# AzheeeQAQ/Game-of-life-distributed

Measured on AMD Instinct MI355X. Metric: cell-updates/sec (GCUPS) at 1/2/4/8 MI355X; % of HBM roofline, higher is better.
Workload: dtype u32 bit-sliced (1 bit/cell)

## Files before the change

### game-of-life-distributed_amd/csrc/gol_kernels.hip

```cpp
#include "gol_kernels.h"
#include "gol_bits.h"
#include "gol_layout.h"

#include <algorithm>
#include <climits>
#include <type_traits>
#include <utility>

namespace golk {
#ifndef GOL_LOOP_PAD
#define GOL_LOOP_PAD 0
#endif
#ifndef GOL_FILL_PHASES
#define GOL_FILL_PHASES 4
#endif

template <typename F, int... I>
__device__ __forceinline__ void static_for_impl(F &&f, std::integer_sequence<int, I...>) {
    (f(std::integral_constant<int, I>()), ...);
}
template <int N, typename F>
__device__ __forceinline__ void static_for(F &&f) {
    static_for_impl(f, std::make_integer_sequence<int, N>());
}
// ... 696 lines not shown
    unit_pr<D, (KQ + 0 + LO) & 1, WPL>(LO, x0, sh, st, x1, nx);
    sh = nx;
    static_for<D - LO>([&](auto t_tag) {
        constexpr int t = LO + decltype(t_tag)::value;
        parity_fix<2>();
        if constexpr (t + 1 < D) {
            unit_pr<D, (KQ + 1 + t) & 1, WPL>(t, x1, sh, st, x0, nx);
            sh = nx;
            unit_pr<D, (KQ + 0 + t + 1) & 1, WPL>(t + 1, x0, sh, st, x2, nx);
            sh = nx;
            unit_pr<D, (KQ + 2 + t) & 1, WPL>(t, x2, sh, st, x1, nx);
            sh = nx;
        } else {
            unit_pr<D, (KQ + 1 + t) & 1, WPL>(t, x1, sh, st, x2, nx);
            sh = nx;
            xn = vmov_even(n0);
            __builtin_amdgcn_sched_barrier(0);
            unit_pr<D, (KQ + 2 + t) & 1, WPL>(t, x2, sh, st, xn, nx);
            sh = nx;
        }
    });
}
template <int D, int KQ, int WPL>
__device__ __forceinline__ void push_group_pr(Lanes<WPL> &x0, Lanes<WPL> &x1, Lanes<WPL> &x2, PairSt<D, WPL> &st,
                                              Shifted &sh, const Lanes<WPL> &n0, Lanes<WPL> &xn) {
    push_group_pr_hi<D, KQ, 0, WPL>(x0, x1, x2, st, sh, n0, xn);
}

template <int D, int KQ, int WPL>
__device__ __forceinline__ void pr_enter(const uint32_t (&h0)[3][D][WPL], const uint32_t (&h1)[3][D][WPL],
                                         const uint32_t (&cc)[3][D][WPL], PairSt<D, WPL> &st) {
#pragma unroll
    for (int t = 0; t < D; ++t)
#pragma unroll
        for (int k = 0; k < WPL; ++k) {
            st.c[t][k] = cc[2][t][k];
            if (((KQ + t) & 1) == 1) {
                st.a0[t][k] = h0[1][t][k];
                st.a1[t][k] = h1[1][t][k];
                st.b0[t][k] = h0[2][t][k];
                st.b1[t][k] = h1[2][t][k];
            } else {
                pair_sum(h0[1][t][k], h1[1][t][k], h0[2][t][k], h1[2][t][k], st.p0[t][k], st.p1[t][k], st.p2[t][k]);
                st.a0[t][k] = h0[2][t][k];
                st.a1[t][k] = h1[2][t][k];
            }
        }
}
template <int D, int KQ, int WPL>
__device__ __forceinline__ void pr_leave(const PairSt<D, WPL> &st, uint32_t (&h0)[3][D][WPL],
                                         uint32_t (&h1)[3][D][WPL], uint32_t (&cc)[3][D][WPL]) {
#pragma unroll
    for (int t = 0; t < D; ++t)
#pragma unroll
        for (int k = 0; k < WPL; ++k) {
            cc[2][t][k] = st.c[t][k];
            if (((KQ + t) & 1) == 1) {
                h0[1][t][k] = st.a0[t][k];
                h1[1][t][k] = st.a1[t][k];
                h0[2][t][k] = st.b0[t][k];
                h1[2][t][k] = st.b1[t][k];
            } else {
                h0[2][t][k] = st.a0[t][k];
                h1[2][t][k] = st.a1[t][k];
                pair_unsum(st.p0[t][k], st.p1[t][k], st.a0[t][k], st.a1[t][k], h0[1][t][k], h1[1][t][k]);
            }
        }
}

template <int D, int LO, int WPL>
__device__ __forceinline__ void push_group_hi(Lanes<WPL> &x0, Lanes<WPL> &x1, Lanes<WPL> &x2,
                                              uint32_t (&h0)[3][D][WPL], uint32_t (&h1)[3][D][WPL],
                                              uint32_t (&cc)[3][D][WPL]) {
    parity_fix<1>();
#pragma unroll
    for (int s = LO; s < D + 2; ++s) {
        parity_fix<2>();
        if (s < D) stage<D, 0, WPL>(s, x0, h0, h1, cc);
        if (s - 1 >= LO && s - 1 < D) stage<D, 1, WPL>(s - 1, x1, h0, h1, cc);
        if (s - 2 >= LO) stage<D, 2, WPL>(s - 2, x2, h0, h1, cc);
    }
}

template <int D, int WPL, bool HALF = false, bool PR = false>
__device__ __forceinline__ uint32_t stream_skew(const StepArgs &a, int ab, int eb, int tile, bool self,
                                                uint32_t *exp_mine, const uint32_t *exp_next, int *flag_mine,
                                                int *flag_next, unsigned *error, unsigned long long *phase_tr,
                                                int dr = 0) {
    using SP = SkewPlan<D>;
    constexpr int ROW = 64 * WPL;
    constexpr int TV = HALF ? kHalfTileValid : kTileValid;
    const int lane = threadIdx.x & 63;
    const int hl = HALF ? (lane & 31) : lane;
    const int rofs = (HALF && lane >= 32) ? dr : 0;
    const int Ww = a.Ww;
    const int S = eb - ab;
    const int t0 = tile * TV * WPL;
    int col = (t0 + WPL * (hl - 1)) % Ww;
    if (col < 0) col += Ww;
    const bool keep = hl >= 1 && hl <= TV && (t0 + WPL * (hl - 1)) < Ww;
    int r = ab + rofs + a.in.off;
    const int wrap = a.in.wrap > 0 ? a.in.wrap : INT_MAX;
    if (a.in.wrap > 0) {
        r %= a.in.wrap;
        if (r < 0) r += a.in.wrap;
    }
    const uint32_t *__restrict__ src = a.src + col;
    auto load_next = [&]() -> Lanes<WPL> {
        const Lanes<WPL> v = load_row<WPL>(src + (size_t)(a.in.base + min(r, a.in.rmax)) * Ww);
        r = (r + 1 == wrap) ? 0 : r + 1;
        return v;
    };
    const __amdgpu_buffer_rsrc_t brs = __builtin_amdgcn_make_buffer_rsrc(
        a.dst + (size_t)(a.dst_base + ab + D) * Ww, (short)0, (S + (HALF ? dr : 0)) * Ww * 4, 0x00020000);
    const int clo = a.count_lo - (ab + D + rofs), chi = a.count_hi - (ab + D + rofs);
    const int colw = col + rofs * Ww;
    uint32_t cnt = 0;
    auto emit = [&](const Lanes<WPL> &y, int oi) {
        const bool ok = keep && (unsigned)oi < (unsigned)S;
        const int off = ok ? (oi * Ww + colw) * 4 : INT_MAX;
        if constexpr (WPL == 1)
            __builtin_amdgcn_raw_buffer_store_b32(y.w[0], brs, off, 0, GOL_SKEW_STORE_CPOL);
        else if constexpr (WPL == 2)
            __builtin_amdgcn_raw_buffer_store_b64((__attribute__((ext_vector_type(2))) unsigned){y.w[0], y.w[1]}, brs,
                                                  off, 0, GOL_SKEW_STORE_CPOL);
        else
            __builtin_amdgcn_raw_buffer_store_b128(
                (__attribute__((ext_vector_type(4))) unsigned){y.w[0], y.w[1], y.w[2], y.w[3]}, brs, off, 0,
                GOL_SKEW_STORE_CPOL);
        uint32_t pc = 0;
#pragma unroll
        for (int k = 0; k < WPL; ++k) pc += __builtin_popcount(y.w[k]);
        cnt += (ok && oi >= clo && oi < chi) ? pc : 0u;
    };
    auto hook = [&](int s, int k, const Lanes<WPL> &x) {
        if (s % SP::STEP != 0 || s == 0 || s / SP::STEP > SP::NPH) return;
        const int j = s / SP::STEP - 1;
        const int m = k - 2 * SP::P(j);
        const int row = (unsigned)m < (unsigned)SP::NROWS(j) ? SP::BASE(j) + m : SP::NEXP;
        put_lanes<WPL>(exp_mine + row * ROW, x.w);
    };

    uint32_t h0[3][D][WPL], h1[3][D][WPL], cc[3][D][WPL];
#pragma unroll
    for (int s = 0; s < 3; ++s)
#pragma unroll
        for (int t = 0; t < D; ++t)
#pragma unroll
            for (int k = 0; k < WPL; ++k) h0[s][t][k] = h1[s][t][k] = cc[s][t][k] = 0u;

    Lanes<WPL> x0 = vmov(load_next()), x1 = vmov(load_next()), x2 = vmov(load_next());
    int k = 0;
    [[maybe_unused]] unsigned long long wt0 = 0, wmain = 0, nmain = 0, wfill = 0, nfill = 0;
    auto fill = [&](auto a_tag) {
        constexpr int A = decltype(a_tag)::value;
        for (; A == D ? k <= 2 * D - 1 : (k + 2) / 2 <= A - 1; k += 3) {
            const Lanes<WPL> n0 = load_next(), n1 = load_next(), n2 = load_next();
            __builtin_amdgcn_sched_barrier(0);
            Lanes<WPL> y0 = x0, y1 = x1, y2 = x2;
            push_group_exp<D, A, WPL>(y0, y1, y2, h0, h1, cc, k, hook);
            if constexpr (A == D) {
                emit(y0, k - 2 * D);
                emit(y1, k + 1 - 2 * D);
                emit(y2, k + 2 - 2 * D);
            }
            __builtin_amdgcn_sched_barrier(0);
            if constexpr (GOL_SKEW_WAIT_TRACE) wt0 = __builtin_amdgcn_s_memrealtime();
            x0 = vmov(n0);
            x1 = vmov(n1);
            x2 = vmov(n2);
            if constexpr (GOL_SKEW_WAIT_TRACE) {
                asm volatile("s_waitcnt vmcnt(0)" ::: "memory");
                wfill += __builtin_amdgcn_s_memrealtime() - wt0;
                ++nfill;
            }
        }
    };
    static_for<SP::NPH>([&](auto j) { fill(std::integral_constant<int, SP::P(decltype(j)::value)>()); });
    fill(std::integral_constant<int, D>());
    if (phase_tr && lane == 0) phase_tr[0] = (unsigned long long)__builtin_amdgcn_s_memrealtime();
    asm volatile("s_waitcnt lgkmcnt(0)" ::: "memory");
    if (lane == 0) __hip_atomic_store(flag_mine, 1, __ATOMIC_RELAXED, __HIP_MEMORY_SCOPE_WORKGROUP);

    Lanes<WPL> q0, q1, q2;
#pragma unroll
    for (int i = 0; i < WPL; ++i) q0.w[i] = q1.w[i] = q2.w[i] = 0u;
    int qoi = -8;
    [[maybe_unused]] PairSt<D, WPL> st;
    [[maybe_unused]] Shifted sh = {0u, 0u};
    const int kmain = S + (self ? 2 * D : 2 * SP::P(0));
    for (int i = 0; i < GOL_LOOP_PAD; ++i) asm volatile("s_nop 0");
    if constexpr (PR) {
        constexpr int KSTART = 3 * ((2 * D + 2) / 3);
        static_assert(KSTART % 6 == 0, "the pair main loop starts at an even push");
        {
            pr_enter<D, 0, WPL>(h0, h1, cc, st);
            sh = row_shifts<WPL>(x0);
            for (; k < kmain; k += 6) {
                {
                    const Lanes<WPL> n0 = load_next(), n1 = load_next(), n2 = load_next();
                    emit(q0, qoi);
                    emit(q1, qoi + 1);
                    emit(q2, qoi + 2);
                    __builtin_amdgcn_sched_barrier(0);
                    Lanes<WPL> y0 = x0, y1 = x1, y2 = x2;
                    Lanes<WPL> xn;
                    push_group_pr<D, 0, WPL>(y0, y1, y2, st, sh, n0, xn);
                    q0 = y0;
                    q1 = y1;
                    q2 = y2;
                    qoi = k - 2 * D;
                    __builtin_amdgcn_sched_barrier(0);
                    x0 = xn;
                    if constexpr (HALF) x1 = vmov(n1); else x1 = vmov_even(n1);
                    x2 = vmov(n2);
                }
// ... 69 lines not shown
            static_for<SP::NPH>([&](auto j) {
                constexpr int J = decltype(j)::value;
                if (J > 0 && d >= 2 * SP::P(J)) base = SP::BASE(J) - 2 * SP::P(J);
            });
            const int top = SP::NEXP - 1;
            y0 = get_lanes<WPL>(exp_next + min(base + d, top) * ROW);
            y1 = get_lanes<WPL>(exp_next + min(base + d + 1, top) * ROW);
            y2 = get_lanes<WPL>(exp_next + min(base + d + 2, top) * ROW);
        };
        {
            Lanes<WPL> n0, n1, n2;
            imports(k, n0, n1, n2);
            x0 = vmov(n0);
            x1 = vmov(n1);
            x2 = vmov(n2);
            if constexpr (PR && D % 3 == 0) sh = row_shifts<WPL>(x0);
        }
        auto drain_pr = [&](auto kq_tag, auto lo_tag) {
            constexpr int KQ = decltype(kq_tag)::value, LO = decltype(lo_tag)::value;
            Lanes<WPL> n0, n1, n2;
            imports(k + 3, n0, n1, n2);
            __builtin_amdgcn_sched_barrier(0);
            Lanes<WPL> y0 = x0, y1 = x1, y2 = x2;
            Lanes<WPL> xn;
            push_group_pr_hi<D, KQ, LO, WPL>(y0, y1, y2, st, sh, n0, xn);
            parity_fix<1>();
            emit(q0, qoi);
            emit(q1, qoi + 1);
            emit(q2, qoi + 2);
            q0 = y0;
            q1 = y1;
            q2 = y2;
            qoi = k - 2 * D;
            __builtin_amdgcn_sched_barrier(0);
            x0 = xn;
            x1 = vmov(n1);
            x2 = vmov(n2);
            k += 3;
        };
        auto drain = [&](auto lo_tag, int kend) {
            constexpr int LO = decltype(lo_tag)::value;
            if constexpr (PR && D % 3 == 0) {
                if constexpr (LO == SP::P(SP::NPH - 1) && D - LO <= 6) {
                    static_for<(D - LO) / 3>([&](auto) {
                        drain_pr(std::integral_constant<int, 0>(), lo_tag);
                        drain_pr(std::integral_constant<int, 1>(), lo_tag);
                    });
                    return;
                }
                while (k < kend) {
                    drain_pr(std::integral_constant<int, 0>(), lo_tag);
                    drain_pr(std::integral_constant<int, 1>(), lo_tag);
                }
                return;
            }
            for (; k < kend; k += 3) {
                Lanes<WPL> n0, n1, n2;
                imports(k + 3, n0, n1, n2);
                __builtin_amdgcn_sched_barrier(0);
                Lanes<WPL> y0 = x0, y1 = x1, y2 = x2;
                push_group_hi<D, LO, WPL>(y0, y1, y2, h0, h1, cc);
                __builtin_amdgcn_sched_barrier(0);
                emit(q0, qoi);
                emit(q1, qoi + 1);
                emit(q2, qoi + 2);
                q0 = y0;
                q1 = y1;
                q2 = y2;
                qoi = k - 2 * D;
                __builtin_amdgcn_sched_barrier(0);
                x0 = vmov(n0);
                x1 = vmov(n1);
                x2 = vmov(n2);
            }
        };
        static_for<SP::NPH>([&](auto j) {
            constexpr int J = decltype(j)::value;
            drain(std::integral_constant<int, SP::P(J)>(), S + 2 * (J + 1 < SP::NPH ? SP::P(J + 1) : D));
        });
    }
    emit(q0, qoi);
    emit(q1, qoi + 1);
    emit(q2, qoi + 2);
    return cnt;
}

template <int D, int WPL, bool HALF = false, bool PR = false>
__global__ __launch_bounds__(512) void gol_skew_kernel(SkewArgs p) {
    using SP = SkewPlan<D>;
    constexpr int ROW = 64 * WPL;
    __shared__ uint32_t s_exp[8][(SP::NEXP + 1) * ROW];
    __shared__ int s_flag[8];
    __shared__ unsigned long long s_cnt;
    const int lane = threadIdx.x & 63;
    const int w = __builtin_amdgcn_readfirstlane(threadIdx.x >> 6);
    const int sy = 8 / p.tx;
    const int tcols = (p.tiles_x + p.tx - 1) / p.tx;
    const int stack = blockIdx.x / tcols, tc = blockIdx.x - stack * tcols;
    const int tile = tc * p.tx + w % p.tx, pos = w / p.tx;
    if (lane == 0) s_flag[w] = 0;
    if (threadIdx.x == 0) s_cnt = 0;
    __syncthreads();
    if (tile >= p.tiles_x) return;
    if (p.prio_young && w >= 4) __builtin_amdgcn_s_setprio(1);
    const int L = HALF ? p.base.rows_out / 2 : p.base.rows_out;
    const int A0 = (int)((int64_t)stack * L / p.nst) - D, E0 = (int)((int64_t)(stack + 1) * L / p.nst) - D;
    const int64_t Ls = (int64_t)(E0 - A0) + p.hcap;
    int cum = 0, tot = 0;
    for (int q = 0; q < sy; ++q) {
        tot += p.wgt[q];
        cum += q < pos ? p.wgt[q] : 0;
    }
    const bool bottom = pos == sy - 1;
    constexpr int G = PR ? 6 : 3;
    const int ab = A0 + (int)(Ls * cum / tot) / G * G;
    const int eb = bottom ? E0 : A0 + (int)(Ls * (cum + p.wgt[pos]) / tot) / G * G;
    const long long t_start = p.trace ? (long long)__builtin_amdgcn_s_memrealtime() : 0;
    const uint32_t cnt = stream_skew<D, WPL, HALF, PR>(p.base, ab, eb, tile, bottom, s_exp[w], bottom ? nullptr : s_exp[w + p.tx],
                                             &s_flag[w], bottom ? nullptr : &s_flag[w + p.tx], p.error,
                                             (p.trace && blockIdx.x < 1024) ? p.trace + 8 + 2 * (blockIdx.x * 64 + 16 + w)
                                                                            : nullptr,
                                             L);
    if (p.trace && lane == 0 && blockIdx.x < 1024) {
        p.trace[8 + 2 * (blockIdx.x * 64 + w)] = (unsigned long long)t_start;
        p.trace[8 + 2 * (blockIdx.x * 64 + w) + 1] = (unsigned long long)__builtin_amdgcn_s_memrealtime();
    }
    if (p.base.alive) wg_count(p.base.alive, &s_cnt, cnt, sy * min(p.tx, p.tiles_x - tc * p.tx));
}

__host__ __device__ constexpr int persist_waves(int depth, int wpl) { return depth * wpl <= 16 ? 16 : 8; }

#ifndef GOL_PERSIST_WG_COUNT
#define GOL_PERSIST_WG_COUNT 1
#endif
template <int D, int WPL, int NW>
__global__ __launch_bounds__(NW * 64) void gol_persist_kernel(PersistArgs p) {
    const int lane = threadIdx.x & 63;
    const int w = __builtin_amdgcn_readfirstlane(threadIdx.x >> 6);
    const int b = blockIdx.x;
    const int wx = b % p.cols, wy = b / p.cols;
    const int tile = wx * p.wg_tx + w % p.wg_tx;
    int r0, band, dir = 1;
    const int ry = w / p.wg_tx;
    const bool paired = p.paired != 0;
    if (paired) {
        const int hr = p.wg_sy / 2;
        r0 = wy * p.wg_sy * p.S + 2 * (ry % hr) * p.S;
        band = 2 * p.S;
        dir = ry < hr ? 1 : -1;
    } else if (p.S_old > 0) {
        const int hr = p.wg_sy / 2;
        const int base = wy * p.wg_sy * p.S;
        r0 = base + (ry < hr ? ry * p.S_old : hr * p.S_old + (ry - hr) * p.S_young);
        band = ry < hr ? p.S_old : p.S_young;
        if (ry == p.wg_sy - 1) band = base + p.wg_sy * p.S - r0;
    } else {
        r0 = (wy * p.wg_sy + ry) * p.S;
        band = p.S;
    }
    const int rows_here = (tile < p.tiles_x && r0 < p.base.rows_out) ? min(band, p.base.rows_out - r0) : 0;

    int nb = b;
    if (lane < 9) {
        const int ny = (wy + lane / 3 - 1 + p.wg_y) % p.wg_y;
        const int nx = (wx + lane % 3 - 1 + p.cols) % p.cols;
        nb = ny * p.cols + nx;
    }
    __shared__ int s_abort;
    __shared__ int s_claim[2][NW / 2];
#if GOL_PERSIST_WG_COUNT
    __shared__ unsigned long long s_cnt;
    if (threadIdx.x == 0) s_cnt = 0;
#endif
    if (threadIdx.x == 0) s_abort = 0;
    if (paired && w < NW / 2 && lane == 0) s_claim[0][w] = rows_here;
    __syncthreads();

    uint32_t cnt = 0;
    long long tr_wait = 0, tr_band = 0, tr_max = 0;
    const long long tr_t0 = (long long)__builtin_amdgcn_s_memrealtime();
    for (int j = 0; j < p.J; ++j) {
        const long long tr_w0 = (long long)__builtin_amdgcn_s_memrealtime();
        if (j > 0) {
            if (w == NW - 1) {
                const long long t_start = (long long)__builtin_amdgcn_s_memrealtime();
                for (;;) {
                    const unsigned v = __hip_atomic_load(&p.progress[nb], __ATOMIC_RELAXED, __HIP_MEMORY_SCOPE_AGENT);
                    if (__all(v >= (unsigned)j)) break;
                    const unsigned err = __hip_atomic_load(p.error, __ATOMIC_RELAXED, __HIP_MEMORY_SCOPE_AGENT);
                    if (err || (long long)__builtin_amdgcn_s_memrealtime() - t_start > p.timeout_ticks) {
                        if (lane == 0) {
                            atomicOr(p.error, 1u);
                            s_abort = 1;
                        }
                        break;
                    }
                    __builtin_amdgcn_s_sleep(2);
                }
                if (lane == 0) __builtin_amdgcn_fence(__ATOMIC_ACQUIRE, "agent");
                asm volatile("s_waitcnt vmcnt(0)" ::: "memory");
            }
            __syncthreads();
            if (s_abort) return;
        }
        const long long tr_b0 = (long long)__builtin_amdgcn_s_memrealtime();
        tr_wait += tr_b0 - tr_w0;
        StepArgs a = p.base;
        const bool odd = ((p.first + j) & 1) != 0;
        a.src = odd ? p.buf1 : p.buf0;
        a.dst = odd ? p.buf0 : p.buf1;
// ... 451 lines not shown
    }
    return n;
}

hipError_t launch_lds_band(const LdsBandArgs &p, int wpl, hipStream_t s) {
    const size_t bytes = (size_t)lds_band_lds_bytes(p.hmax, p.D, p.stride);
    const int S = p.rt_stride ? 0 : lds_tmpl_stride(wpl, p.nt, p.stride);
    if (p.stride != lds_band_stride(p.Ww, wpl, p.nt)) return hipErrorInvalidValue;
    return dispatch_lds_band(wpl, p.nt, S, [&](auto kern, int t) {
        hipLaunchKernelGGL(kern, dim3(p.nb), dim3(t), bytes, s, p);
        return hipGetLastError();
    });
}

template <typename F>
static hipError_t dispatch(int depth, bool skip, int wpl, F &&f) {
#define GOL_CASE(D, SK, WP) \
    if (depth == D && skip == SK && wpl == WP) return f(gol_tb_kernel<D, SK, WP>);
    GOL_CASE(1, true, 1) GOL_CASE(2, true, 1) GOL_CASE(4, true, 1) GOL_CASE(8, true, 1) GOL_CASE(16, true, 1)
    GOL_CASE(32, true, 1) GOL_CASE(1, false, 1) GOL_CASE(2, false, 1) GOL_CASE(4, false, 1) GOL_CASE(8, false, 1)
    GOL_CASE(16, false, 1) GOL_CASE(32, false, 1)
    GOL_CASE(12, true, 1) GOL_CASE(24, true, 1) GOL_CASE(12, false, 1) GOL_CASE(24, false, 1)
    GOL_CASE(12, true, 2) GOL_CASE(12, false, 2)
    GOL_CASE(1, true, 4) GOL_CASE(2, true, 4) GOL_CASE(4, true, 4) GOL_CASE(8, true, 4) GOL_CASE(9, true, 4)
    GOL_CASE(1, false, 4) GOL_CASE(2, false, 4) GOL_CASE(4, false, 4) GOL_CASE(8, false, 4) GOL_CASE(9, false, 4)
    GOL_CASE(6, true, 1) GOL_CASE(6, false, 1) GOL_CASE(6, true, 2) GOL_CASE(6, false, 2)
    GOL_CASE(6, true, 4) GOL_CASE(6, false, 4)
    GOL_CASE(1, true, 2) GOL_CASE(2, true, 2) GOL_CASE(4, true, 2) GOL_CASE(8, true, 2) GOL_CASE(16, true, 2)
    GOL_CASE(1, false, 2) GOL_CASE(2, false, 2) GOL_CASE(4, false, 2) GOL_CASE(8, false, 2) GOL_CASE(16, false, 2)
    GOL_CASE(20, true, 1) GOL_CASE(20, false, 1) GOL_CASE(20, true, 2) GOL_CASE(20, false, 2)
    GOL_CASE(18, true, 2) GOL_CASE(18, false, 2)
#undef GOL_CASE
    return hipErrorInvalidValue;
}

int max_depth_for(int wpl) { return wpl == 4 ? 9 : wpl == 2 ? 20 : 32; }
int persist_max_depth(int wpl) { return wpl == 4 ? 8 : wpl == 2 ? 16 : 32; }

int tb_tiles(int Ww, int wpl) { return (Ww + tile_words(wpl) - 1) / tile_words(wpl); }

int tb_waves(const StepArgs &a, int wpl) {
    const int strips = (a.rows_out + a.rows_per_wave - 1) / a.rows_per_wave;
    return tb_tiles(a.Ww, wpl) * strips;
}

template <typename F>
static hipError_t dispatch_pair(int depth, int wpl, F &&f, bool cnt = false) {
#define GOL_QCASE(D, WP) \
    if (depth == D && wpl == WP) return cnt ? f(gol_tb_pair_kernel<D, WP, true>) : f(gol_tb_pair_kernel<D, WP, false>);
    GOL_QCASE(1, 1) GOL_QCASE(2, 1) GOL_QCASE(4, 1) GOL_QCASE(8, 1) GOL_QCASE(16, 1) GOL_QCASE(32, 1)
    GOL_QCASE(1, 2) GOL_QCASE(2, 2) GOL_QCASE(4, 2) GOL_QCASE(8, 2) GOL_QCASE(16, 2)
    GOL_QCASE(12, 1) GOL_QCASE(24, 1) GOL_QCASE(12, 2) GOL_QCASE(1, 4) GOL_QCASE(2, 4) GOL_QCASE(4, 4) GOL_QCASE(8, 4)
    GOL_QCASE(6, 1) GOL_QCASE(6, 2) GOL_QCASE(6, 4) GOL_QCASE(9, 4) GOL_QCASE(20, 1) GOL_QCASE(20, 2)
    GOL_QCASE(18, 2)
#undef GOL_QCASE
    return hipErrorInvalidValue;
}

int tb_pair_blocks(const StepArgs &a, int wpl) {
    const int regions = (a.rows_out + 2 * a.rows_per_wave - 1) / (2 * a.rows_per_wave);
    return (tb_tiles(a.Ww, wpl) * regions + 3) / 4;
}

hipError_t launch_step_tb(const StepArgs &a, int depth, hipStream_t s, bool fill_skip, int wpl, bool paired) {
    if (paired && fill_skip) {
        const dim3 grid(tb_pair_blocks(a, wpl)), block(512);
        return dispatch_pair(
            depth, wpl,
            [&](auto kern) {
                hipLaunchKernelGGL(kern, grid, block, 0, s, a);
                return hipGetLastError();
            },
            a.alive != nullptr);
    }
    const int waves = tb_waves(a, wpl);
    const dim3 grid((waves + 3) / 4), block(256);
    return dispatch(depth, fill_skip, wpl, [&](auto kern) {
        hipLaunchKernelGGL(kern, grid, block, 0, s, a);
        return hipGetLastError();
    });
}

template <typename F>
static hipError_t dispatch_skew(int depth, int wpl, bool half, bool pr, F &&f) {
#define GOL_WCASE(D, WP) \
    if (!pr && !half && depth == D && wpl == WP) return f(gol_skew_kernel<D, WP>);
#define GOL_HCASE(D, WP) \
    if (!pr && half && depth == D && wpl == WP) return f(gol_skew_kernel<D, WP, true>);
#define GOL_RCASE(D, WP, HF) \
    if (pr && half == HF && depth == D && wpl == WP) return f(gol_skew_kernel<D, WP, HF, true>);
    GOL_WCASE(8, 2) GOL_WCASE(12, 2) GOL_WCASE(16, 2) GOL_WCASE(20, 2) GOL_WCASE(6, 4) GOL_WCASE(8, 4)
    GOL_WCASE(9, 4) GOL_WCASE(16, 1) GOL_WCASE(32, 1)
    GOL_HCASE(16, 2) GOL_HCASE(20, 2)
    GOL_RCASE(18, 2, false) GOL_RCASE(18, 2, true) GOL_RCASE(8, 4, false)
#undef GOL_WCASE
#undef GOL_HCASE
#undef GOL_RCASE
    return hipErrorInvalidValue;
}

bool skew_supported(int depth, int wpl, bool half, bool pr) {
    return dispatch_skew(depth, wpl, half, pr, [](auto) { return hipSuccess; }) == hipSuccess;
}

int skew_blocks_per_cu(int depth, int wpl, bool half, bool pr) {
    int b = 0;
    hipError_t e = dispatch_skew(depth, wpl, half, pr, [&](auto kern) {
        return hipOccupancyMaxActiveBlocksPerMultiprocessor(&b, kern, 512, 0);
    });
    return e == hipSuccess ? b : 0;
}

hipError_t launch_skew(const SkewArgs &p, int depth, int wpl, hipStream_t s) {
    const int tcols = (p.tiles_x + p.tx - 1) / p.tx;
    return dispatch_skew(depth, wpl, p.half != 0, p.pairs != 0, [&](auto kern) {
        hipLaunchKernelGGL(kern, dim3(tcols * p.nst), dim3(512), 0, s, p);
        return hipGetLastError();
    });
}

int tb_blocks_per_cu(int depth, int wpl) {
    int b = 0;
    hipError_t e = dispatch(depth, true, wpl, [&](auto kern) {
        return hipOccupancyMaxActiveBlocksPerMultiprocessor(&b, kern, 256, 0);
    });
    return (e == hipSuccess && b > 0) ? b : 1;
}

int tb_wave_slots_per_cu(int depth, int wpl, bool paired) {
    if (!paired) return 4 * tb_blocks_per_cu(depth, wpl);
    int b = 0;
    hipError_t e = dispatch_pair(depth, wpl, [&](auto kern) {
        return hipOccupancyMaxActiveBlocksPerMultiprocessor(&b, kern, 512, 0);
    });
    return 8 * ((e == hipSuccess && b > 0) ? b : 1);
}

int auto_rows_per_wave(int Ww, int rows, int depth, int wave_slots, bool fill_skip, int wpl, bool paired) {
    const int tiles_x = tb_tiles(Ww, wpl);
    int best_s = rows;
    double best = 1e300;
    for (int strips = 1; strips <= rows; ++strips) {
        const int S = (rows + strips - 1) / strips;
        const long long waves = paired ? 2LL * tiles_x * ((rows + 2 * S - 1) / (2 * S))
                                       : (long long)tiles_x * ((rows + S - 1) / S);
        const long long rounds = (waves + wave_slots - 1) / wave_slots;
        const double cost = (double)rounds * (S + (fill_skip ? 2 * depth - 0.75 * depth : 2 * depth));
        if (cost < best * 0.999) {
            best = cost;
            best_s = S;
        }
        if (S <= 2) break;
    }
    return best_s;
}

template <typename F>
static hipError_t dispatch_persist(int depth, int wpl, int nw, F &&f) {
    if (nw == 0) nw = persist_waves(depth, wpl);
#define GOL_PCASE(D, WP, NW) \
    if (depth == D && wpl == WP && nw == NW) return f(gol_persist_kernel<D, WP, NW>, NW);
    GOL_PCASE(4, 1, 16) GOL_PCASE(8, 1, 16) GOL_PCASE(16, 1, 16) GOL_PCASE(32, 1, 8) GOL_PCASE(4, 2, 16)
    GOL_PCASE(8, 2, 16) GOL_PCASE(16, 2, 8) GOL_PCASE(8, 1, 8) GOL_PCASE(16, 1, 8) GOL_PCASE(8, 2, 8)
#undef GOL_PCASE
    return hipErrorInvalidValue;
}

int persist_waves_for(int depth, int wpl) { return persist_waves(depth, wpl); }

int persist_blocks_per_cu(int depth, int wpl, int nw) {
    int b = 0;
    hipError_t e = dispatch_persist(depth, wpl, nw, [&](auto kern, int n) {
        return hipOccupancyMaxActiveBlocksPerMultiprocessor(&b, kern, 64 * n, 0);
    });
    return e == hipSuccess ? b : 0;
}

bool plan_persist(int Ww, int rows, int depth, int cus, int wpl, int units, PersistArgs *p, int force_tx) {
    const int NW = units;
    const int tiles_x = tb_tiles(Ww, wpl);
    bool found = false;
    long best_s = 0;
    for (int wg_tx = 1; wg_tx <= NW; wg_tx *= 2) {
        if (force_tx > 0 && wg_tx != force_tx) continue;
        const int wg_sy = NW / wg_tx;
        const int cols = (tiles_x + wg_tx - 1) / wg_tx;
        int wg_y = std::min(cus / cols, rows / (wg_sy * depth));
        if (wg_y < 1) continue;
        const int strips = wg_y * wg_sy;
        const int S = (rows + strips - 1) / strips;
        if (S < depth) continue;
        wg_y = (rows + wg_sy * S - 1) / (wg_sy * S);
        const int last_rows = rows - (wg_y - 1) * wg_sy * S;
        if (last_rows < depth) continue;
        if (!found || S < best_s) {
            found = true;
            best_s = S;
            p->wg_tx = wg_tx;
// ... 986 lines not shown
```

### game-of-life-distributed_amd/csrc/golhip_plan.cpp

```cpp
#include "golhip_impl.h"
#include <climits>
#include <functional>

namespace gh GOLHIP_HIDDEN {

int largest_depth(int64_t want) {
    for (int d : kDepths)
        if (d <= want && d != 9 && d != 18) return d;
    return 1;
}
static bool special_depth(int d) { return d == 9 || d == 18; }

DepthRun depth_plan(int cap, int64_t left) {
    const int M = special_depth(cap) ? cap : largest_depth(std::max(1, cap));
    if (left <= 0) return {M, 0};
    const int64_t head = std::max<int64_t>(0, left / M - 12);
    const int t = (int)(left - head * M);
    std::vector<int> nl(t + 1, INT_MAX), mn(t + 1, 0), pick(t + 1, 0);
    nl[0] = 0;
    mn[0] = INT_MAX;
    for (int v = 1; v <= t; ++v)
        for (int d : kDepths) {
            if (d > M || d > v || nl[v - d] == INT_MAX || (special_depth(d) && M != d)) continue;
            const int n = nl[v - d] + 1, m = std::min(mn[v - d], d);
// ... 74 lines not shown
}

int want_il(golhip_t h) { return wpl_for(h) >= 2 ? wpl_for(h) : 0; }

int depth_cap(golhip_t h, bool halo) {
    if (h->W % 32 != 0) return 1;
    const int wpl = wpl_for(h);
    int cap = std::min(h->tb_depth, (halo && persist_on(h)) ? golk::persist_max_depth(wpl) : golk::max_depth_for(wpl));
    if (halo) cap = std::min(cap, sched_rows(h));
    bool pair = false;
    if ((h->skew_pairs & 1) && wpl == 2 && cap >= 18) {
        golk::SkewArgs sk{};
        if (skew_dims(h, 18, 2, halo ? sched_rows(h) : h->rows, &sk) && (!sk.half || (h->skew_pairs & 4))) {
            cap = 18;
            pair = true;
        }
    }
    if (!pair && !halo && wpl == 2 && cap > 16) {
        golk::SkewArgs sk{};
        if (skew_dims(h, 20, 2, h->rows, &sk) && sk.half) cap = 16;
    }
    if (cap == 9 && (wpl != 4 || (halo && persist_on(h)))) cap = 8;
    if (cap == 18 && !pair) cap = 16;
    if ((h->skew_pairs & 2) && wpl == 4 && cap >= 8) {
        golk::SkewArgs sk{};
        if (skew_dims(h, 8, 4, halo ? sched_rows(h) : h->rows, &sk) && !sk.half) cap = 8;
    }
    return cap;
}

int next_depth(golhip_t h, int64_t remaining, bool halo) { return depth_plan(depth_cap(h, halo), remaining).d; }

static int depth_index(int d) {
    for (int i = 0; i < kNumDepths; ++i)
        if (kDepths[i] == d) return i;
    return kNumDepths - 1;
}

bool tb_paired(golhip_t h) { return h->paired_bands && h->fill_skip; }

int rows_per_wave_for(golhip_t h, int depth) {
    if (h->rows_per_wave > 0) return h->rows_per_wave;
    int &c = h->auto_rpw[depth_index(depth)];
    if (c == 0) {
        const int wpl = wpl_for(h);
        const int slots = h->cu_count * golk::tb_wave_slots_per_cu(depth, wpl, tb_paired(h));
        c = golk::auto_rows_per_wave(h->Ww, h->rows, depth, std::max(slots, 1), h->fill_skip, wpl, tb_paired(h));
    }
    return c;
}

void halo_plan(int strip_rows, int nranks, int rank, int depth, int Ww, golhip_halo_plan_t *p) {
    p->prev_rank = (rank - 1 + nranks) % nranks;
    p->next_rank = (rank + 1) % nranks;
    p->rows = depth;
    p->send_up_row = kHalo;
    p->recv_bottom_row = kHalo + strip_rows;
    p->send_down_row = kHalo + strip_rows - depth;
    p->recv_top_row = kHalo - depth;
    p->bytes = (int64_t)depth * Ww * 4;
}

static int skew_bpc(golhip_t h, int depth, int wpl, bool half, bool pr) {
    int &c = h->skew_bpc[depth_index(depth)][(wpl == 4 ? 2 : wpl - 1) + (half ? 3 : 0) + (pr ? 6 : 0)];
    if (c == 0) {
        const int b = golk::skew_blocks_per_cu(depth, wpl, half, pr);
        c = b > 0 ? b : -1;
    }
    return c;
}

bool skew_dims(golhip_t h, int depth, int wpl, int L, golk::SkewArgs *sk) {
    const bool pr = (depth == 18 && (h->skew_pairs & 1)) || (wpl == 4 && depth == 8 && (h->skew_pairs & 2));
    if (!h->skew || h->W % 32 != 0 || !golk::skew_supported(depth, wpl, false, pr)) return false;
    const int hcap = h->skew_hcap >= 0 ? h->skew_hcap : 3 * depth / 4;
    const int smin = depth + 3;
    const bool half_ok = h->skew_half >= 0 && L % 2 == 0 && golk::skew_supported(depth, wpl, true, pr);
    int best_tx = 0, best_nst = 0, best_half = 0, best_tiles = 0;
    double best = 1e300;
    for (int half = 0; half <= (half_ok ? 1 : 0); ++half) {
        if (!half && half_ok && h->skew_half > 0) continue;
        const int bpc = skew_bpc(h, depth, wpl, half, pr);
        if (bpc < 1) continue;
        const int tiles = half ? (h->Ww + golk::kHalfTileValid * wpl - 1) / (golk::kHalfTileValid * wpl)
                               : golk::tb_tiles(h->Ww, wpl);
        const int Lh = half ? L / 2 : L;
        for (int tx = 1; tx <= 2; ++tx) {
            if (h->skew_tx && tx != h->skew_tx) continue;
            const int sy = 8 / tx, tcols = (tiles + tx - 1) / tx;
            const int nst = std::min(h->cu_count * bpc / tcols,
                                     Lh / (sy * (smin + hcap) - hcap));
            if (nst < 1) continue;
            if (h->skew == 1 && (int64_t)nst * tcols * 4 < (int64_t)h->cu_count * bpc * 3) continue;
            if (((double)Lh / nst + hcap + (half ? Lh : 0)) * h->Ww * 4 >= 2147483648.0) continue;
            const double per_wave = ((double)Lh / nst + hcap) / sy * (half ? 1.02 : 1.0);
            if (per_wave < best * 0.999) {
                best = per_wave;
                best_tx = tx;
                best_nst = nst;
                best_half = half;
                best_tiles = tiles;
            }
        }
    }
    if (!best_tx) return false;
    sk->tiles_x = best_tiles;
    sk->pairs = pr ? 1 : 0;
    sk->tx = best_tx;
    sk->nst = best_nst;
    sk->half = best_half;
    sk->hcap = hcap;
    return true;
}

static bool skew_fills(golhip_t h) {
    if (!h->skew || h->W % 32 != 0) return false;
    const int wpl = wpl_per_launch(h);
    int cap = std::min(h->tb_depth, golk::max_depth_for(wpl));
    if (cap == 9 && wpl != 4) cap = 8;
    const int depth = cap == 9 ? 9 : largest_depth(cap);
    golk::SkewArgs sk{};
    return skew_dims(h, depth, wpl, sched_rows(h), &sk);
}

bool skew_plan(golhip_t h, int depth, int wpl, const golk::StepArgs &a, golk::SkewArgs *sk) {
    if (!skew_dims(h, depth, wpl, a.rows_out, sk)) return false;
    if (!h->skew_err) {
        void *p = nullptr, *d = nullptr;
        if (hipHostMalloc(&p, sizeof(unsigned), hipHostMallocMapped) != hipSuccess) return false;
        if (hipHostGetDevicePointer(&d, p, 0) != hipSuccess) {
            (void)hipHostFree(p);
            return false;
        }
        h->skew_err = static_cast<unsigned *>(p);
        h->skew_err_dev = static_cast<unsigned *>(d);
        *h->skew_err = 0;
    }
    const int sy = 8 / sk->tx;
    const int young = h->skew_young > 0 ? h->skew_young
                      : wpl == 4             ? 78
                      : sk->half             ? 60
                      : a.in.wrap > 0        ? (sk->pairs ? 80 : 70)
                                             : 68;
    for (int q = 0; q < 8; ++q) sk->wgt[q] = (q < sy && q * sk->tx >= 4) ? young : 100;
    sk->prio_young = h->skew_prio;
    sk->error = h->skew_err_dev;
    sk->trace = h->d_trace;
    return true;
}

int halo_launches(int rows, int depth, int64_t run) {
    const int64_t k = std::min<int64_t>({(int64_t)kHalo / depth, run, (int64_t)rows / depth});
    return (int)std::max<int64_t>(1, k);
}

HaloRun halo_next(int cap, int rows, bool resident, int64_t left) {
    DepthRun run = depth_plan(cap, left);
    if (resident) {
        const int d = largest_depth(std::min<int64_t>(cap, left));
        run = {d, left / d};
    }
    return {run.d, halo_launches(rows, run.d, run.n)};
}

int persist_depth_for(golhip_t h, int wpl) {
    const int cap = std::min(h->persist_depth > 0 ? h->persist_depth : h->tb_depth, golk::persist_max_depth(wpl));
// ... 78 lines not shown
```

Before: 146,100.

## Add count-free skew kernel variants and cheaper scalar/buffer row addressing

Adds a CNT template flag so skew kernels compiled without an alive-count pointer skip the per-row popcounts and the workgroup count reduction. Row loading is rewritten to keep the source row base in scalar registers, advanced with s_cmp/s_cselect wrap handling, while HALF kernels use buffer loads with a per-half offset update through v_add3. Store offsets are precomputed to cut per-emit VALU work. This adds template instantiations, inline asm and a planner guard that excludes half mode when the grid exceeds 4 GiB, since buffer offsets are 32-bit.

Result: no change. 147,300, median of 6 (+0.8%).

```diff
diff --git a/game-of-life-distributed_amd/csrc/gol_kernels.hip b/game-of-life-distributed_amd/csrc/gol_kernels.hip
--- a/game-of-life-distributed_amd/csrc/gol_kernels.hip
+++ b/game-of-life-distributed_amd/csrc/gol_kernels.hip
@@ -802,7 +802,39 @@
     }
 }
 
-template <int D, int WPL, bool HALF = false, bool PR = false>
+__device__ __forceinline__ uint64_t sel_eq_u64(uint64_t a, uint64_t b, uint64_t t, uint64_t f) {
+    uint64_t r;
+    asm("s_cmp_eq_u64 %1, %2\n\ts_cselect_b64 %0, %3, %4" : "=s"(r) : "s"(a), "s"(b), "s"(t), "s"(f) : "scc");
+    return r;
+}
+
+template <int WPL>
+__device__ __forceinline__ Lanes<WPL> load_row_at(uint64_t row, uint32_t off) {
+    typedef const __attribute__((address_space(1))) char *gbytes;
+    typedef __attribute__((address_space(1))) uint32_t gword;
+    typedef unsigned word2 __attribute__((ext_vector_type(2)));
+    typedef unsigned word4 __attribute__((ext_vector_type(4)));
+    typedef __attribute__((address_space(1))) word2 gword2;
+    typedef __attribute__((address_space(1))) word4 gword4;
+    const gbytes p = reinterpret_cast<gbytes>(row) + off;
+    Lanes<WPL> v;
+    if constexpr (WPL == 1) {
+        v.w[0] = *reinterpret_cast<const gword *>(p);
+    } else if constexpr (WPL == 2) {
+        const word2 q = *reinterpret_cast<const gword2 *>(p);
+        v.w[0] = q.x;
+        v.w[1] = q.y;
+    } else {
+        const word4 q = *reinterpret_cast<const gword4 *>(p);
+        v.w[0] = q.x;
+        v.w[1] = q.y;
+        v.w[2] = q.z;
+        v.w[3] = q.w;
+    }
+    return v;
+}
+
+template <int D, int WPL, bool HALF = false, bool PR = false, bool CNT = true>
 __device__ __forceinline__ uint32_t stream_skew(const StepArgs &a, int ab, int eb, int tile, bool self,
                                                 uint32_t *exp_mine, const uint32_t *exp_next, int *flag_mine,
                                                 int *flag_next, unsigned *error, unsigned long long *phase_tr,
@@ -819,26 +851,65 @@
     int col = (t0 + WPL * (hl - 1)) % Ww;
     if (col < 0) col += Ww;
     const bool keep = hl >= 1 && hl <= TV && (t0 + WPL * (hl - 1)) < Ww;
-    int r = ab + rofs + a.in.off;
+    const uint32_t Wb = (uint32_t)Ww * 4u;
     const int wrap = a.in.wrap > 0 ? a.in.wrap : INT_MAX;
-    if (a.in.wrap > 0) {
-        r %= a.in.wrap;
-        if (r < 0) r += a.in.wrap;
-    }
-    const uint32_t *__restrict__ src = a.src + col;
+    const int rlast = min(a.in.rmax, wrap - 1);
+    auto mapped = [&](int r) {
+        if (a.in.wrap > 0) {
+            r %= a.in.wrap;
+            if (r < 0) r += a.in.wrap;
+        }
+        return min(r, a.in.rmax);
+    };
+    const uint32_t *const row0 = a.src + (size_t)a.in.base * Ww;
+    [[maybe_unused]] uint64_t sb = (uint64_t)row0 + (uint64_t)mapped(ab + a.in.off) * Wb;
+    [[maybe_unused]] const uint64_t sb_last = (uint64_t)row0 + (uint64_t)rlast * Wb;
+    [[maybe_unused]] const uint64_t sb_next = a.in.wrap > 0 ? (uint64_t)row0 : sb_last;
+    [[maybe_unused]] uint32_t lvoff = (uint32_t)col * 4u;
+    [[maybe_unused]] uint32_t so0 = (uint32_t)mapped(ab + a.in.off) * Wb, so1 = (uint32_t)mapped(ab + dr + a.in.off) * Wb;
+    [[maybe_unused]] const uint32_t so_last = (uint32_t)rlast * Wb, so_jump = a.in.wrap > 0 ? 0u - so_last : 0u;
+    [[maybe_unused]] uint32_t upper = (HALF && lane >= 32) ? ~0u : 0u;
+    if constexpr (HALF) asm volatile("v_mov_b32 %0, %0" : "+v"(upper));
+    [[maybe_unused]] uint32_t vo = lvoff + so0 + (upper & (so1 - so0));
+    [[maybe_unused]] const __amdgpu_buffer_rsrc_t lrs = __builtin_amdgcn_make_buffer_rsrc(
+        const_cast<uint32_t *>(row0), (short)0, HALF ? (rlast + 1) * Wb : 0u, 0x00020000);
     auto load_next = [&]() -> Lanes<WPL> {
-        const Lanes<WPL> v = load_row<WPL>(src + (size_t)(a.in.base + min(r, a.in.rmax)) * Ww);
-        r = (r + 1 == wrap) ? 0 : r + 1;
+        Lanes<WPL> v;
+        if constexpr (HALF) {
+            if constexpr (WPL == 1) {
+                v.w[0] = __builtin_amdgcn_raw_buffer_load_b32(lrs, vo, 0, 0);
+            } else if constexpr (WPL == 2) {
+                const auto q = __builtin_amdgcn_raw_buffer_load_b64(lrs, vo, 0, 0);
+                v.w[0] = q[0];
+                v.w[1] = q[1];
+            } else {
+                const auto q = __builtin_amdgcn_raw_buffer_load_b128(lrs, vo, 0, 0);
+                v.w[0] = q[0];
+                v.w[1] = q[1];
+                v.w[2] = q[2];
+                v.w[3] = q[3];
+            }
+            const uint32_t st0 = so0 == so_last ? so_jump : Wb, st1 = so1 == so_last ? so_jump : Wb;
+            so0 += st0;
+            so1 += st1;
+            const uint32_t du = upper & (st1 - st0);
+            asm volatile("v_add3_u32 %0, %0, %1, %2" : "+v"(vo) : "s"(st0), "v"(du));
+        } else {
+            asm volatile("" : "+v"(lvoff));
+            v = load_row_at<WPL>(sb, lvoff);
+            sb = sel_eq_u64(sb, sb_last, sb_next, sb + Wb);
+        }
         return v;
     };
     const __amdgpu_buffer_rsrc_t brs = __builtin_amdgcn_make_buffer_rsrc(
         a.dst + (size_t)(a.dst_base + ab + D) * Ww, (short)0, (S + (HALF ? dr : 0)) * Ww * 4, 0x00020000);
     const int clo = a.count_lo - (ab + D + rofs), chi = a.count_hi - (ab + D + rofs);
     const int colw = col + rofs * Ww;
-    uint32_t cnt = 0;
+    const uint32_t svoff = keep ? (uint32_t)colw * 4u : (uint32_t)INT_MAX;
+    [[maybe_unused]] uint32_t cnt = 0;
     auto emit = [&](const Lanes<WPL> &y, int oi) {
-        const bool ok = keep && (unsigned)oi < (unsigned)S;
-        const int off = ok ? (oi * Ww + colw) * 4 : INT_MAX;
+        const bool rok = (unsigned)oi < (unsigned)S;
+        const uint32_t off = svoff + (rok ? (uint32_t)oi * Wb : (uint32_t)INT_MAX);
         if constexpr (WPL == 1)
             __builtin_amdgcn_raw_buffer_store_b32(y.w[0], brs, off, 0, GOL_SKEW_STORE_CPOL);
         else if constexpr (WPL == 2)
@@ -848,10 +919,12 @@
             __builtin_amdgcn_raw_buffer_store_b128(
                 (__attribute__((ext_vector_type(4))) unsigned){y.w[0], y.w[1], y.w[2], y.w[3]}, brs, off, 0,
                 GOL_SKEW_STORE_CPOL);
-        uint32_t pc = 0;
-#pragma unroll
-        for (int k = 0; k < WPL; ++k) pc += __builtin_popcount(y.w[k]);
-        cnt += (ok && oi >= clo && oi < chi) ? pc : 0u;
+        if constexpr (CNT) {
+            uint32_t pc = 0;
+#pragma unroll
+            for (int k = 0; k < WPL; ++k) pc += __builtin_popcount(y.w[k]);
+            cnt += (keep && rok && oi >= clo && oi < chi) ? pc : 0u;
+        }
     };
     auto hook = [&](int s, int k, const Lanes<WPL> &x) {
         if (s % SP::STEP != 0 || s == 0 || s / SP::STEP > SP::NPH) return;
@@ -1087,16 +1160,17 @@
     emit(q0, qoi);
     emit(q1, qoi + 1);
     emit(q2, qoi + 2);
-    return cnt;
-}
-
-template <int D, int WPL, bool HALF = false, bool PR = false>
+    if constexpr (CNT) return cnt;
+    return 0u;
+}
+
+template <int D, int WPL, bool HALF = false, bool PR = false, bool CNT = true>
 __global__ __launch_bounds__(512) void gol_skew_kernel(SkewArgs p) {
     using SP = SkewPlan<D>;
     constexpr int ROW = 64 * WPL;
     __shared__ uint32_t s_exp[8][(SP::NEXP + 1) * ROW];
     __shared__ int s_flag[8];
-    __shared__ unsigned long long s_cnt;
+    [[maybe_unused]] __shared__ unsigned long long s_cnt;
     const int lane = threadIdx.x & 63;
     const int w = __builtin_amdgcn_readfirstlane(threadIdx.x >> 6);
     const int sy = 8 / p.tx;
@@ -1104,7 +1178,7 @@
     const int stack = blockIdx.x / tcols, tc = blockIdx.x - stack * tcols;
     const int tile = tc * p.tx + w % p.tx, pos = w / p.tx;
     if (lane == 0) s_flag[w] = 0;
-    if (threadIdx.x == 0) s_cnt = 0;
+    if (CNT && threadIdx.x == 0) s_cnt = 0;
     __syncthreads();
     if (tile >= p.tiles_x) return;
     if (p.prio_young && w >= 4) __builtin_amdgcn_s_setprio(1);
@@ -1121,7 +1195,7 @@
     const int ab = A0 + (int)(Ls * cum / tot) / G * G;
     const int eb = bottom ? E0 : A0 + (int)(Ls * (cum + p.wgt[pos]) / tot) / G * G;
     const long long t_start = p.trace ? (long long)__builtin_amdgcn_s_memrealtime() : 0;
-    const uint32_t cnt = stream_skew<D, WPL, HALF, PR>(p.base, ab, eb, tile, bottom, s_exp[w], bottom ? nullptr : s_exp[w + p.tx],
+    [[maybe_unused]] const uint32_t cnt = stream_skew<D, WPL, HALF, PR, CNT>(p.base, ab, eb, tile, bottom, s_exp[w], bottom ? nullptr : s_exp[w + p.tx],
                                              &s_flag[w], bottom ? nullptr : &s_flag[w + p.tx], p.error,
                                              (p.trace && blockIdx.x < 1024) ? p.trace + 8 + 2 * (blockIdx.x * 64 + 16 + w)
                                                                             : nullptr,
@@ -1130,7 +1204,9 @@
         p.trace[8 + 2 * (blockIdx.x * 64 + w)] = (unsigned long long)t_start;
         p.trace[8 + 2 * (blockIdx.x * 64 + w) + 1] = (unsigned long long)__builtin_amdgcn_s_memrealtime();
     }
-    if (p.base.alive) wg_count(p.base.alive, &s_cnt, cnt, sy * min(p.tx, p.tiles_x - tc * p.tx));
+    if constexpr (CNT) {
+        if (p.base.alive) wg_count(p.base.alive, &s_cnt, cnt, sy * min(p.tx, p.tiles_x - tc * p.tx));
+    }
 }
 
 __host__ __device__ constexpr int persist_waves(int depth, int wpl) { return depth * wpl <= 16 ? 16 : 8; }
@@ -1748,30 +1824,38 @@
 }
 
 template <typename F>
-static hipError_t dispatch_skew(int depth, int wpl, bool half, bool pr, F &&f) {
+static hipError_t dispatch_skew(int depth, int wpl, bool half, bool pr, bool cnt, F &&f) {
 #define GOL_WCASE(D, WP) \
-    if (!pr && !half && depth == D && wpl == WP) return f(gol_skew_kernel<D, WP>);
+    if (cnt && !pr && !half && depth == D && wpl == WP) return f(gol_skew_kernel<D, WP>);
 #define GOL_HCASE(D, WP) \
-    if (!pr && half && depth == D && wpl == WP) return f(gol_skew_kernel<D, WP, true>);
+    if (cnt && !pr && half && depth == D && wpl == WP) return f(gol_skew_kernel<D, WP, true>);
 #define GOL_RCASE(D, WP, HF) \
-    if (pr && half == HF && depth == D && wpl == WP) return f(gol_skew_kernel<D, WP, HF, true>);
+    if (cnt && pr && half == HF && depth == D && wpl == WP) return f(gol_skew_kernel<D, WP, HF, true>);
+#define GOL_NCASE(D, WP, HF, PR) \
+    if (!cnt && pr == PR && half == HF && depth == D && wpl == WP) return f(gol_skew_kernel<D, WP, HF, PR, false>);
     GOL_WCASE(8, 2) GOL_WCASE(12, 2) GOL_WCASE(16, 2) GOL_WCASE(20, 2) GOL_WCASE(6, 4) GOL_WCASE(8, 4)
     GOL_WCASE(9, 4) GOL_WCASE(16, 1) GOL_WCASE(32, 1)
     GOL_HCASE(16, 2) GOL_HCASE(20, 2)
     GOL_RCASE(18, 2, false) GOL_RCASE(18, 2, true) GOL_RCASE(8, 4, false)
+    GOL_NCASE(8, 2, false, false) GOL_NCASE(12, 2, false, false) GOL_NCASE(16, 2, false, false)
+    GOL_NCASE(20, 2, false, false) GOL_NCASE(6, 4, false, false) GOL_NCASE(8, 4, false, false)
+    GOL_NCASE(9, 4, false, false) GOL_NCASE(16, 1, false, false) GOL_NCASE(32, 1, false, false)
+    GOL_NCASE(16, 2, true, false) GOL_NCASE(20, 2, true, false)
+    GOL_NCASE(18, 2, false, true) GOL_NCASE(18, 2, true, true) GOL_NCASE(8, 4, false, true)
 #undef GOL_WCASE
 #undef GOL_HCASE
 #undef GOL_RCASE
+#undef GOL_NCASE
     return hipErrorInvalidValue;
 }
 
 bool skew_supported(int depth, int wpl, bool half, bool pr) {
-    return dispatch_skew(depth, wpl, half, pr, [](auto) { return hipSuccess; }) == hipSuccess;
+    return dispatch_skew(depth, wpl, half, pr, true, [](auto) { return hipSuccess; }) == hipSuccess;
 }
 
 int skew_blocks_per_cu(int depth, int wpl, bool half, bool pr) {
     int b = 0;
-    hipError_t e = dispatch_skew(depth, wpl, half, pr, [&](auto kern) {
+    hipError_t e = dispatch_skew(depth, wpl, half, pr, true, [&](auto kern) {
         return hipOccupancyMaxActiveBlocksPerMultiprocessor(&b, kern, 512, 0);
     });
     return e == hipSuccess ? b : 0;
@@ -1779,7 +1863,7 @@
 
 hipError_t launch_skew(const SkewArgs &p, int depth, int wpl, hipStream_t s) {
     const int tcols = (p.tiles_x + p.tx - 1) / p.tx;
-    return dispatch_skew(depth, wpl, p.half != 0, p.pairs != 0, [&](auto kern) {
+    return dispatch_skew(depth, wpl, p.half != 0, p.pairs != 0, p.base.alive != nullptr, [&](auto kern) {
         hipLaunchKernelGGL(kern, dim3(tcols * p.nst), dim3(512), 0, s, p);
         return hipGetLastError();
     });
diff --git a/game-of-life-distributed_amd/csrc/golhip_plan.cpp b/game-of-life-distributed_amd/csrc/golhip_plan.cpp
--- a/game-of-life-distributed_amd/csrc/golhip_plan.cpp
+++ b/game-of-life-distributed_amd/csrc/golhip_plan.cpp
@@ -180,6 +180,7 @@
         if (!half && half_ok && h->skew_half > 0) continue;
         const int bpc = skew_bpc(h, depth, wpl, half, pr);
         if (bpc < 1) continue;
+        if (half && (double)h->phys_rows * h->Ww * 4 >= 4294967296.0) continue;
         const int tiles = half ? (h->Ww + golk::kHalfTileValid * wpl - 1) / (golk::kHalfTileValid * wpl)
                                : golk::tb_tiles(h->Ww, wpl);
         const int Lh = half ? L / 2 : L;
```
